# pyamg/pyamg

Measured on AMD Instinct MI355X. Metric: vcycle_iterations_per_sec, higher is better.
Workload: dtype f64; 1 GPU; 3D 7-pt Poisson 256^3 (16.7M dof) SA V-cycle, symmetric Gauss-Seidel, fp64; key=c3, n=16777216, nnz=117047296, levels=5, cycle=V(1,1), graph=True, parallelism=1 GPU, gs_order=fast, full=False

## Files before the change

### pyamg_amd/_build.py

```python
from __future__ import annotations

import os
import shutil
import subprocess
import sys
from concurrent.futures import ThreadPoolExecutor
from pathlib import Path

PKG = Path(__file__).resolve().parent
CSRC = PKG / "csrc"
LIB = PKG / "libpyamg_amd.so"
SOURCES = ["pamg_matrix.hip", "pamg_solver.hip", "pamg_capi.hip", "pamg_setup.hip", "pamg_schwarz.hip", "pamg_dist.hip", "pamg_aggregate.hip", "pamg_lane.hip", "pamg_line.hip", "pamg_kz.hip", "pamg_blane.hip", "pamg_block.hip", "pamg_renumber.hip", "pamg_krylov.hip", "pamg_schwarz_setup.hip", "pamg_classical.hip", "pamg_air.hip"]
HEADERS = ["pamg_common.h", "pamg_kernels.h", "pamg_tile_kernels.h", "pamg_tile_plan.h", "pamg_lane_plan.h", "pamg_lanem_plan.h", "pamg_schwarz_plan.h", "pamg_line_plan.h", "pamg_kz_plan.h", "pamg_blane_plan.h", "pamg_spg_plan.h", "pamg_stream_plan.h", "pamg_rowmask_map.h", "pamg_plan_vec.h", "pamg_host_threads.h", "pamg_dense_pinv.h", "pamg_classical.h", "pamg_air.h", "amg_core_bind.cpp", "../../include/pyamg_amd.h"]
FLAGS = ["--offload-arch=gfx950", "-O3", "-std=c++17", "-fPIC", "-ffp-contract=off",
         "-fno-fast-math", "-Wall", "-Wno-unused-function", "-Wno-unused-value", "-Wno-unused-result"]


def hipcc() -> str:
    for c in (os.environ.get("HIPCC"), shutil.which("hipcc"), "/opt/rocm/bin/hipcc"):
        if c and Path(c).exists():
            return c
    raise RuntimeError("hipcc not found (need ROCm's hipcc to build libpyamg_amd.so)")


def stale() -> bool:
    if not LIB.exists():
        return True
    try:
# ... 63 lines not shown
```

### pyamg_amd/csrc/pamg_common.h

```cpp
#pragma once
#include "pamg_host_threads.h"
#include <hip/hip_runtime.h>

#include <cstdint>
#include <cstdio>
#include <cstdlib>
#include <ctime>
#include <algorithm>
#include <atomic>
#include <cstring>
#include <thread>
#include <vector>

#include "../../include/pyamg_amd.h"

#define PAMG_STR2(x) #x
#define PAMG_STR(x) PAMG_STR2(x)
#define PAMG_HIP(expr)                                   \
    do {                                                 \
        hipError_t e__ = (expr);                         \
        if (e__ != hipSuccess) return (int)e__;          \
    } while (0)
#define PAMG_TRY(expr)                                   \
    do {                                                 \
// ... 200 lines not shown
    int sym_cap = 0;
    const void *sym_cap_kernel = nullptr;
    int zsym_cap = 0;
    const void *zsym_cap_kernel = nullptr;
    int csym_cap = 0;
    const void *csym_cap_kernel = nullptr;
    int sym_general_grid = 0;
    int sym_form = 0, sym_grid = 0;
    long long sym_launches = 0, sym_zero_launches = 0;
    int zero_plans = 0;
    int zero_merge = 0;
    struct pamg::LaneMSched *zplan[2] = {nullptr, nullptr};
    void *d_zw = nullptr;
    size_t zero_bytes = 0;
    long long zero_plan_launches = 0;
    int gs_correction = 0;
    long long correction_launches = 0;
    size_t bytes = 0;
};

struct pamg_schwarz_s;
struct pamg_solver_s;
struct pamg_csr_s;

namespace pamg {
int schwarz_sweep(pamg_schwarz_s *h, void *x, const void *b, int start, int stop, int step, hipStream_t s);
int schwarz_prepare(pamg_schwarz_s *h, int sweep);
int schwarz_error(pamg_schwarz_s *h, bool *error);
void schwarz_level_launches(pamg_schwarz_s *h);
int schwarz_blocks_device(int dtype, pamg_matrix_s *A, int nsub, const int *d_Sp, const int *d_Sj, int *d_Tp, void *d_Tx,
// ... 96 lines not shown
size_t lanem_part_bytes(const GsSchedule *g);
int lanem_info(const GsSchedule *g, int64_t *info, double *growth);
int lanem_levels(const GsSchedule *g, int64_t *out, int64_t cap, int64_t *n);
int lanem_sym_launch(pamg_matrix_s *A, GsSchedule *gf, GsSchedule *gb, void *x, const void *b, bool x_zero, hipStream_t s, bool acc = false);
int lanem_plan_info(const struct LaneMSched *t, int64_t *info, double *growth);
int build_zero_plan(pamg_matrix_s *A, int dir);
void free_zero_plans(pamg_matrix_s *A);
size_t zero_plan_bytes(const pamg_matrix_s *A);
bool zero_plans_ready(const pamg_matrix_s *A, const GsSchedule *gf, const GsSchedule *gb);
int lanem_zero_pair_launch(pamg_matrix_s *A, GsSchedule *gf, GsSchedule *gb, void *x, const void *b, bool acc, hipStream_t s);
int ensure_zero_parts(pamg_matrix_s *A, bool build);
void matrix_drop_zero_plans(pamg_matrix_s *A);
int gs_sweep_zero_pair(pamg_matrix_s *A, void *x, const void *b, hipStream_t s, bool *ran);
int gs_sweep_correction(pamg_matrix_s *A, void *x, const void *b, void *r, bool force, hipStream_t s, bool *ran);
constexpr int64_t GS_CORRECTION_MIN_ROWS = 16384;
int sym_fill_sentinels(void *p, int64_t n);
int sweep_error(pamg_matrix_s *A, bool *error);
inline size_t tsize(int dtype) { return dtype == PAMG_F64 ? 8 : 4; }

template <typename F>
inline void host_parallel(int64_t n, F fn, int64_t grain = 1 << 20)
{
    const unsigned hw = std::max(1u, std::min(32u, pamg::host_cpus()));
    const int nt = n < 2 * grain ? 1 : (int)std::min<int64_t>(hw, n / grain);
    if (nt <= 1) { fn((int64_t)0, n); return; }
    std::vector<std::thread> th;
    for (int t = 0; t < nt; ++t) {
        const int64_t lo = n * t / nt, hi = n * (t + 1) / nt;
        th.emplace_back([=] { fn(lo, hi); });
    }
// ... 19 lines not shown
```

### pyamg_amd/csrc/pamg_lane.hip

```cpp
#include "pamg_common.h"
#include "pamg_lane_plan.h"
#include "pamg_lanem_plan.h"
#include "pamg_tile_plan.h"

namespace pamg {

template <typename T> struct Sentinel;
template <> struct Sentinel<double> {
    using bits_t = unsigned long long;
    static constexpr bits_t value = 0x7FF8DEADBEEF5A5Aull;
    static __device__ __forceinline__ bits_t bits(double v) { return (bits_t)__double_as_longlong(v); }
};
template <> struct Sentinel<float> {
    using bits_t = unsigned int;
    static constexpr bits_t value = 0x7FC5BEEFu;
    static __device__ __forceinline__ bits_t bits(float v) { return __float_as_uint(v); }
};

template <typename T>
__global__ __launch_bounds__(BLK) void lane_fill_sentinel_kernel(T *xs, int64_t n)
{
    using B = typename Sentinel<T>::bits_t;
    B *p = reinterpret_cast<B *>(xs);
    for (int64_t i = (int64_t)blockIdx.x * BLK + threadIdx.x; i < n; i += (int64_t)gridDim.x * BLK) p[i] = Sentinel<T>::value;
// ... 301 lines not shown
    const void *cap_kernel = nullptr;
    size_t bytes = 0;
};

struct LaneMArgs {
    const int *cols;
    const double *vals;
    const LaneMRec *rec;
    const double *xold;
    double *y;
    double *xs;
    const double *b;
    unsigned *err;
    unsigned *ticket;
    int ngroups, nidle, use_gate;
    long long *prof;
    const unsigned short *sidx;
    const int *crid;
    const double *crd;
    int crows;
    double *w;
};

__global__ __launch_bounds__(BLK) void lanem_prepare_kernel(const double *__restrict__ x, double *__restrict__ xold, double *__restrict__ xs, int64_t n)
{
    unsigned long long *p = reinterpret_cast<unsigned long long *>(xs);
    for (int64_t i = (int64_t)blockIdx.x * BLK + threadIdx.x; i < n; i += (int64_t)gridDim.x * BLK) {
        xold[i] = x[i];
        p[i] = Sentinel<double>::value;
    }
// ... 272 lines not shown
    const T num = bv - s;
    T val = num * rd;
    if (!upd) val = xo;
    if (tail && rid >= 0) {
        __hip_atomic_store(a.xs + row, val, __ATOMIC_RELAXED, __HIP_MEMORY_SCOPE_AGENT);
        if constexpr (PH != 1) {
            if (upd) {
                if constexpr (ACC) a.y[row] = a.y[row] + val;
                else a.y[row] = val;
            }
        }
        if constexpr (WST) {
            if (upd) __hip_atomic_store(a.w + row, num, __ATOMIC_RELAXED, __HIP_MEMORY_SCOPE_AGENT);
        }
    }
}

template <int MODE, int RPW, int NREG, int Z = 0>
__global__ __launch_bounds__(BLK) void gs_lanem_kernel(const LaneMArgs a)
{
    const int lane = threadIdx.x & 63;
    const int wib = threadIdx.x >> 6;
    const int idle = (int)((((unsigned)blockIdx.x * LANE_WPB + (unsigned)wib) * 16u) % (unsigned)a.nidle);
    const int4 *rp = reinterpret_cast<const int4 *>(a.rec);
    const int gend = a.ngroups;
    __shared__ double c_lds[RPW == 0 ? LANE_WPB * LANEC_UMAX : 1];
    if constexpr (RPW == 0) {
        static_assert(RPW != 0 || MODE != 1, "the cluster layout has no ticket form");
        const int W = (int)gridDim.x * LANE_WPB;
        int g = __builtin_amdgcn_readfirstlane((int)blockIdx.x * LANE_WPB + wib);
// ... 28 lines not shown
                if (lane == 0) {
                    long long *o = a.prof + (size_t)g * 4;
                    o[0] = t0 | ((long long)(sp > 4095u ? 4095u : sp) << 52);
                    o[1] = t1; o[2] = t2; o[3] = wall_clock64();
                }
            } else {
                m_slots<RPW, NREG>(a, X, q0, q1, g, lane);
                m_gather<NREG>(a, X, idle);
                const double val = m_finish<RPW, NREG>(a, X, idle);
                m_publish<RPW, MODE, NREG, 0, Z == 1, Z == 2>(a, X, val);
            }
            q0 = n0; q1 = n1;
        }
    } else {
        __shared__ int sh_home;
        if (threadIdx.x == 0) {
            const unsigned me = (__builtin_amdgcn_s_getreg((3 << 11) | 20) & 0xF) + 1u;
            unsigned home = 0u;
            __hip_atomic_compare_exchange_strong(a.ticket + 1, &home, me, __ATOMIC_RELAXED, __ATOMIC_RELAXED, __HIP_MEMORY_SCOPE_AGENT);
            sh_home = (home == 0u || home == me) ? 1 : 0;
        }
        __syncthreads();
        if (!sh_home) return;
        unsigned tk = 0;
        if (lane == 0) tk = __hip_atomic_fetch_add(a.ticket, 1u, __ATOMIC_RELAXED, __HIP_MEMORY_SCOPE_AGENT);
        int g = (int)__builtin_amdgcn_readfirstlane(tk);
        if (g >= gend) return;
        if (lane == 0) tk = __hip_atomic_fetch_add(a.ticket, 1u, __ATOMIC_RELAXED, __HIP_MEMORY_SCOPE_AGENT);
        int g2 = (int)__builtin_amdgcn_readfirstlane(tk);
        int4 q0, q1;
        m_rec(rp, g, gend, q0, q1);
        while (true) {
            int4 n0, n1;
            m_rec(rp, g2, gend, n0, n1);
            unsigned tk3 = 0;
            if (g2 < gend && lane == 0) tk3 = __hip_atomic_fetch_add(a.ticket, 1u, __ATOMIC_RELAXED, __HIP_MEMORY_SCOPE_AGENT);
            m_slots<RPW, NREG>(a, X, q0, q1, g, lane);
            m_gather<NREG>(a, X, idle);
            const double val = m_finish<RPW, NREG>(a, X, idle);
            m_publish<RPW, MODE, NREG, 0, Z == 1, Z == 2>(a, X, val);
            if (g2 >= gend) break;
            g = g2; q0 = n0; q1 = n1;
            g2 = (int)__builtin_amdgcn_readfirstlane(tk3);
        }
    }
    }
}

struct LaneMSymArgs {
    LaneMArgs ph[2];
    double *hf[2];
    unsigned *sync;
    int wq[2], wr[2], wblk[2];
    int xzero;
};

template <int MODE>
__device__ __forceinline__ void m_wipe(double *w, int g, int G, int q, int r, int blk, int lane)
{
    if (g & (blk - 1)) return;
    const int g1 = g + blk < G ? g + blk : G;
    const int lo = g * q + (g < r ? g : r), hi = g1 * q + (g1 < r ? g1 : r);
    unsigned long long *p = reinterpret_cast<unsigned long long *>(w);
    for (int i = lo + lane; i < hi; i += 64) {
        if constexpr (MODE == 1) __hip_atomic_store(p + i, Sentinel<double>::value, __ATOMIC_RELAXED, __HIP_MEMORY_SCOPE_WORKGROUP);
        else __hip_atomic_store(p + i, Sentinel<double>::value, __ATOMIC_RELAXED, __HIP_MEMORY_SCOPE_AGENT);
    }
}

template <int MODE, int RPW, int NREG, int PH, int Z = 0>
__device__ __forceinline__ unsigned m_phase(const LaneMArgs &a, double *wipe, int wq, int wr, int wblk, unsigned *ticket, const bool xz, int lane, int wib, int idle, double *c_lds)
{
    const int4 *rp = reinterpret_cast<const int4 *>(a.rec);
    const int gend = a.ngroups;
    unsigned done = 0;
    if constexpr (RPW == 0) {
        static_assert(RPW != 0 || MODE != 1, "the cluster layout has no ticket form");
        const int W = (int)gridDim.x * LANE_WPB;
        int g = __builtin_amdgcn_readfirstlane((int)blockIdx.x * LANE_WPB + wib);
        if (g >= gend) return 0;
        int4 q = c_rec(rp, g, gend);
        for (; g < gend; g += W) {
            const int4 nq = c_rec(rp, g + W, gend);
            c_group<PH, Z && PH == 1, Z && PH == 2, Z == 2>(a, c_lds + wib * LANEC_UMAX, q, g, lane, idle, xz, PH == 2);
            m_wipe<MODE>(wipe, g, gend, wq, wr, wblk, lane);
            ++done;
// ... 7 lines not shown
        if (g >= gend) return 0;
        int4 q0, q1;
        m_rec(rp, g, gend, q0, q1);
        for (; g < gend; g += W) {
            int4 n0, n1;
            m_rec(rp, g + W, gend, n0, n1);
            m_slots<RPW, NREG>(a, X, q0, q1, g, lane);
            m_gather<NREG, Z && PH == 2, Z == 2 && PH == 1>(a, X, idle, xz, PH == 2);
            const double val = m_finish<RPW, NREG>(a, X, idle, nullptr, nullptr, xz);
            m_publish<RPW, MODE, NREG, PH, Z && PH == 1, Z == 2 && PH == 2>(a, X, val);
            m_wipe<MODE>(wipe, g, gend, wq, wr, wblk, lane);
            ++done;
            q0 = n0; q1 = n1;
        }
    } else {
        unsigned tk = 0;
        if (lane == 0) tk = __hip_atomic_fetch_add(ticket, 1u, __ATOMIC_RELAXED, __HIP_MEMORY_SCOPE_AGENT);
        int g = (int)__builtin_amdgcn_readfirstlane(tk);
        if (g >= gend) return 0;
        if (lane == 0) tk = __hip_atomic_fetch_add(ticket, 1u, __ATOMIC_RELAXED, __HIP_MEMORY_SCOPE_AGENT);
        int g2 = (int)__builtin_amdgcn_readfirstlane(tk);
        int4 q0, q1;
        m_rec(rp, g, gend, q0, q1);
        while (true) {
            int4 n0, n1;
            m_rec(rp, g2, gend, n0, n1);
            unsigned tk3 = 0;
            if (g2 < gend && lane == 0) tk3 = __hip_atomic_fetch_add(ticket, 1u, __ATOMIC_RELAXED, __HIP_MEMORY_SCOPE_AGENT);
            m_slots<RPW, NREG>(a, X, q0, q1, g, lane);
            m_gather<NREG, Z && PH == 2, Z == 2 && PH == 1>(a, X, idle, xz, PH == 2);
            const double val = m_finish<RPW, NREG>(a, X, idle, nullptr, nullptr, xz);
            m_publish<RPW, MODE, NREG, PH, Z && PH == 1, Z == 2 && PH == 2>(a, X, val);
            m_wipe<MODE>(wipe, g, gend, wq, wr, wblk, lane);
            ++done;
            if (g2 >= gend) break;
            g = g2; q0 = n0; q1 = n1;
            g2 = (int)__builtin_amdgcn_readfirstlane(tk3);
        }
    }
    }
    return done;
}

__device__ __forceinline__ void sym_phase_barrier(unsigned *counter, unsigned *err, unsigned *sh_done, unsigned done, unsigned total)
{
    asm volatile("s_waitcnt vmcnt(0)" ::: "memory");
    if ((threadIdx.x & 63) == 0 && done) atomicAdd(sh_done, done);
    __syncthreads();
    if (threadIdx.x == 0) {
        const unsigned mine = *sh_done;
        if (mine) __hip_atomic_fetch_add(counter, mine, __ATOMIC_RELAXED, __HIP_MEMORY_SCOPE_AGENT);
        unsigned spins = 0;
// ... 13 lines not shown
    __syncthreads();
    if (threadIdx.x == 0) {
        const unsigned left = __hip_atomic_fetch_add(sync + 1, 1u, __ATOMIC_RELAXED, __HIP_MEMORY_SCOPE_AGENT);
        if (left == gridDim.x - 1) {
            for (int k = 0; k < 5; ++k) __hip_atomic_store(sync + k, 0u, __ATOMIC_RELAXED, __HIP_MEMORY_SCOPE_AGENT);
            __hip_atomic_store(sync + 5, parity ^ 1u, __ATOMIC_RELAXED, __HIP_MEMORY_SCOPE_AGENT);
        }
    }
}

template <int MODE, int RPW, int NREG, int Z = 0>
__global__ __launch_bounds__(BLK) void gs_lanem_sym_kernel(const LaneMSymArgs a)
{
    __shared__ unsigned sh_done;
    __shared__ int sh_home;
    __shared__ double c_lds[RPW == 0 ? LANE_WPB * LANEC_UMAX : 1];
    const int lane = threadIdx.x & 63;
    const int wib = threadIdx.x >> 6;
    const int idle = (int)((((unsigned)blockIdx.x * LANE_WPB + (unsigned)wib) * 16u) % (unsigned)a.ph[0].nidle);
    const unsigned parity = __builtin_amdgcn_readfirstlane(__hip_atomic_load(a.sync + 5, __ATOMIC_RELAXED, __HIP_MEMORY_SCOPE_AGENT)) & 1u;
    if (threadIdx.x == 0) {
        sh_done = 0u;
        sh_home = 1;
        if constexpr (MODE == 1) {
            const unsigned me = (__builtin_amdgcn_s_getreg((3 << 11) | 20) & 0xF) + 1u;
            unsigned home = 0u;
            __hip_atomic_compare_exchange_strong(a.sync + 4, &home, me, __ATOMIC_RELAXED, __ATOMIC_RELAXED, __HIP_MEMORY_SCOPE_AGENT);
            sh_home = (home == 0u || home == me) ? 1 : 0;
        }
    }
    __syncthreads();
    if (sh_home) {
        double *hf = a.hf[parity], *hf_next = a.hf[parity ^ 1u];
        LaneMArgs p1 = a.ph[0], p2 = a.ph[1];
        p1.xs = hf; p1.y = nullptr;
        p2.xold = hf;
        const unsigned done = m_phase<MODE, RPW, NREG, 1, Z>(p1, p2.xs, a.wq[0], a.wr[0], a.wblk[0], a.sync + 2, a.xzero != 0, lane, wib, idle, c_lds);
        sym_phase_barrier(a.sync, p1.err, &sh_done, done, (unsigned)p1.ngroups);
        (void)m_phase<MODE, RPW, NREG, 2, Z>(p2, hf_next, a.wq[1], a.wr[1], a.wblk[1], a.sync + 3, false, lane, wib, idle, c_lds);
    }
    sym_leave(a.sync, parity);
}

namespace {

template <typename U>
int lane_upload(U **dst, const void *src, size_t bytes, size_t *total)
{
    *dst = nullptr;
    const size_t alloc = std::max<size_t>(bytes, 256) + 256;
    PAMG_HIP(hipMalloc((void **)dst, alloc));
    if (bytes && src) PAMG_HIP(hipMemcpy(*dst, src, bytes, hipMemcpyHostToDevice));
    if (total) *total += alloc;
    return PAMG_OK;
// ... 350 lines not shown
bool zero_plans_ready(const pamg_matrix_s *A, const GsSchedule *gf, const GsSchedule *gb)
{
    const LaneMSched *zf = A->zplan[0], *zb = A->zplan[1];
    if (A->zero_plans == 1 || !zf || !zb || !A->d_zw || !gf || !gb || !gf->lanem || !gb->lanem) return false;
    return zf->rpw == zb->rpw && zf->cluster == zb->cluster && zf->rpw == gf->lanem->rpw && zf->cluster == gf->lanem->cluster &&
           zb->rpw == gb->lanem->rpw && zb->cluster == gb->lanem->cluster && zf->ngroups >= 1 && zb->ngroups >= 1;
}

static void lanem_layout_args(const LaneMSched *t, LaneMArgs &a)
{
    a.cols = t->d_cols; a.vals = t->d_vals;
    a.rec = t->cluster ? reinterpret_cast<const LaneMRec *>(t->d_crec) : t->d_rec;
    a.sidx = t->d_sidx; a.crid = t->d_crid; a.crd = t->d_crd; a.crows = t->cluster;
}

static int lanem_launch_plan(pamg_matrix_s *A, GsSchedule *g, LaneMSched *t, void *x, const void *b, double *w, hipStream_t s, bool acc = false)
{
    if (!t || !g->d_xold) return PAMG_E_STATE;
    const int64_t n = A->nrows;
    LaneMArgs a;
    lanem_layout_args(t, a);
    a.use_gate = (A->lane_flags & 1) ? 1 : 0;
    a.xold = (const double *)g->d_xold; a.y = (double *)x; a.xs = (double *)g->d_xs; a.b = (const double *)b;
    a.w = w;
    a.err = g->d_sync + 1; a.ticket = g->d_sync + 20;
    a.ngroups = (int)t->ngroups;
    a.nidle = (int)std::max<int64_t>(1, std::min<int64_t>(n, 1 << 20));
    if (A->gs_prof && !t->d_prof && !t->cluster) {
        PAMG_HIP(hipMalloc((void **)&t->d_prof, (size_t)t->ngroups * 4 * sizeof(long long)));
        PAMG_HIP(hipMemset(t->d_prof, 0, (size_t)t->ngroups * 4 * sizeof(long long)));
    }
    a.prof = (A->gs_prof && !t->cluster) ? t->d_prof : nullptr;
    const int fgrid = (int)std::min<int64_t>(4096, (n + BLK - 1) / BLK);
    if (acc) hipLaunchKernelGGL((lane_fill_sentinel_kernel<double>), dim3(fgrid), dim3(BLK), 0, s, (double *)g->d_xs, n);
    else hipLaunchKernelGGL(lanem_prepare_kernel, dim3(fgrid), dim3(BLK), 0, s, (const double *)x, (double *)g->d_xold, (double *)g->d_xs, n);
    PAMG_HIP(hipGetLastError());
    const bool xcd = !t->cluster && (A->gran_xcd == 1 || (A->gran_xcd == 0 && lane_one_xcd(A, g) && A->nrows <= 8192));
    static const int nreg_env = [] { const char *e = getenv("PAMG_LANEM_NREG"); return e ? atoi(e) : 0; }();
    const bool all_regs = t->rpw == 1 && (nreg_env ? nreg_env == 8 : A->nrows <= 131072);
    const void *k = t->cluster  ? (const void *)gs_lanem_kernel<0, 0, 8>
                  : t->rpw == 2 ? (xcd ? (const void *)gs_lanem_kernel<1, 2, 4> : (const void *)gs_lanem_kernel<0, 2, 4>)
                  : all_regs    ? (xcd ? (const void *)gs_lanem_kernel<1, 1, 8> : (const void *)gs_lanem_kernel<0, 1, 8>)
                                : (xcd ? (const void *)gs_lanem_kernel<1, 1, 2> : (const void *)gs_lanem_kernel<0, 1, 2>);
    if (w)
        k = t->cluster  ? (const void *)gs_lanem_kernel<0, 0, 8, 1>
          : t->rpw == 2 ? (xcd ? (const void *)gs_lanem_kernel<1, 2, 4, 1> : (const void *)gs_lanem_kernel<0, 2, 4, 1>)
          : all_regs    ? (xcd ? (const void *)gs_lanem_kernel<1, 1, 8, 1> : (const void *)gs_lanem_kernel<0, 1, 8, 1>)
                        : (xcd ? (const void *)gs_lanem_kernel<1, 1, 2, 1> : (const void *)gs_lanem_kernel<0, 1, 2, 1>);
    if (acc)
        k = t->cluster  ? (const void *)gs_lanem_kernel<0, 0, 8, 2>
          : t->rpw == 2 ? (xcd ? (const void *)gs_lanem_kernel<1, 2, 4, 2> : (const void *)gs_lanem_kernel<0, 2, 4, 2>)
          : all_regs    ? (xcd ? (const void *)gs_lanem_kernel<1, 1, 8, 2> : (const void *)gs_lanem_kernel<0, 1, 8, 2>)
// ... 51 lines not shown
    hipLaunchKernelGGL((lane_fill_sentinel_kernel<double>), dim3(fgrid), dim3(BLK), 0, 0, (double *)p, n);
    PAMG_HIP(hipGetLastError());
    PAMG_HIP(hipDeviceSynchronize());
    return PAMG_OK;
}

int lanem_sym_launch(pamg_matrix_s *A, GsSchedule *gf, GsSchedule *gb, void *x, const void *b, bool x_zero, hipStream_t s, bool acc)
{
    LaneMSched *tf = gf->lanem, *tb = gb->lanem;
    if (!tf || !tb || !A->d_sym_hf[0] || !A->d_sym_hf[1] || !A->d_sym_hb || !A->d_sym_sync) return PAMG_E_STATE;
    if (acc && !zero_plans_ready(A, gf, gb)) return PAMG_E_UNSUPPORTED;
    if (acc) x_zero = true;
    const bool zero = x_zero && zero_plans_ready(A, gf, gb);
    if (zero) { tf = A->zplan[0]; tb = A->zplan[1]; }
    const int64_t n = A->nrows;
    auto one_xcd = [&](const GsSchedule *g) { return !g->lanem->cluster && (A->gran_xcd == 1 || (A->gran_xcd == 0 && lane_one_xcd(A, g) && A->nrows <= 8192)); };
    const bool xcd = one_xcd(gf);
    if (xcd != one_xcd(gb) || tf->rpw != tb->rpw || tf->cluster != tb->cluster || tf->ngroups < 1 || tb->ngroups < 1) return PAMG_E_UNSUPPORTED;
    LaneMSymArgs a;
    LaneMSched *ts2[2] = {tf, tb};
    for (int p = 0; p < 2; ++p) {
        LaneMSched *t = ts2[p];
        LaneMArgs &q = a.ph[p];
        lanem_layout_args(t, q);
        q.use_gate = (A->lane_flags & 1) ? 1 : 0;
        q.b = (const double *)b;
        q.w = nullptr;
        q.err = gf->d_sync + 1; q.ticket = nullptr;
        q.ngroups = (int)t->ngroups;
        q.nidle = (int)std::max<int64_t>(1, std::min<int64_t>(n, 1 << 20));
        q.prof = nullptr;
        a.wq[p] = (int)(n / t->ngroups); a.wr[p] = (int)(n % t->ngroups);
        a.wblk[p] = 1;
        while ((int64_t)a.wblk[p] * n < 64 * t->ngroups && a.wblk[p] < (1 << 20)) a.wblk[p] *= 2;
    }
    a.ph[0].xold = (const double *)x; a.ph[0].y = nullptr;     a.ph[0].xs = nullptr;
    a.ph[1].xold = nullptr;           a.ph[1].y = (double *)x; a.ph[1].xs = (double *)A->d_sym_hb;
    if (zero) { a.ph[0].w = (double *)A->d_zw; a.ph[1].b = (const double *)A->d_zw; }
    a.hf[0] = (double *)A->d_sym_hf[0]; a.hf[1] = (double *)A->d_sym_hf[1];
    a.sync = A->d_sym_sync;
    a.xzero = x_zero ? 1 : 0;
    static const int nreg_env = [] { const char *e = getenv("PAMG_LANEM_NREG"); return e ? atoi(e) : 0; }();
    const bool all_regs = tf->rpw == 1 && (nreg_env ? nreg_env == 8 : A->nrows <= 131072);
    const void *k = tf->cluster  ? (const void *)gs_lanem_sym_kernel<0, 0, 8>
// ... 174 lines not shown
```

### pyamg_amd/csrc/pamg_matrix.hip

```cpp
#include "pamg_host_threads.h"
#include <algorithm>
#include <atomic>
#include <mutex>
#include <climits>
#include <new>
#include <thread>

#include "pamg_kernels.h"
#include "pamg_tile_kernels.h"
#include "pamg_tile_plan.h"
#include "pamg_stream_plan.h"

using namespace pamg;

namespace {

constexpr int PAD = 8;

std::mutex g_sched_mu;

template <typename U>
int upload(U **dptr, const U *h, size_t n, size_t *bytes)
{
    const size_t sz = (n + PAD) * sizeof(U);
// ... 1061 lines not shown
    int r0, r1, rs;
    if (A->gs_order != 1 || A->gs_mode != 0 || A->R != A->C || A->point_twin_unfit || !point_twin_bounds(A, g, r0, r1, rs)) return PAMG_OK;
    static std::mutex twin_mu;
    {
        std::lock_guard<std::mutex> lk(twin_mu);
        if (A->point_twin_unfit) return PAMG_OK;
        if (!A->point_twin) {
            PhaseTimer pt_("point twin of a block operator", A->nnz);
            std::vector<unsigned char> hAx((size_t)A->nnz * tsize(A->dtype));
            if (A->nnz) PAMG_HIP(hipMemcpy(hAx.data(), A->d_Ax, hAx.size(), hipMemcpyDeviceToHost));
            pamg_matrix_s *T = nullptr;
            const int st = pamg_matrix_create(&T, A->dtype, PAMG_CSR, (int)A->nrows, (int)A->ncols, 1, 1, A->h_Ap.data(), A->h_Aj.data(), hAx.data());
            if (st != PAMG_OK) { A->point_twin_unfit = true; return st == PAMG_E_UNSUPPORTED || st == PAMG_E_ARG ? PAMG_OK : st; }
            T->gs_order = 1;
            T->lane_L = A->lane_L; T->lane_G = A->lane_G; T->lane_flags = A->lane_flags; T->lane_merge = A->lane_merge; T->line_scan = A->line_scan;
            T->lane_wide = A->lane_wide; T->lanem_rpw = A->lanem_rpw; T->lanem_cluster = A->lanem_cluster; T->lanem_ahead10 = A->lanem_ahead10; T->gran_xcd = A->gran_xcd;
            A->point_twin = T;
            { std::lock_guard<std::mutex> lk2(g_sched_mu); A->bytes += T->bytes; A->point_twin_bytes = T->bytes; }
        }
    }
    GsSchedule *tg = nullptr;
    PAMG_TRY(get_schedule(A->point_twin, r0, r1, rs, &tg));
    PAMG_TRY(ensure_parts(A->point_twin, tg, false));
    if (!tg->lane && !tg->lanem && !tg->line) {
        std::lock_guard<std::mutex> lk(twin_mu);
        A->point_twin_unfit = true;
    }
    return PAMG_OK;
}

int ensure_parts(pamg_matrix_s *A, GsSchedule *g, bool block_gs)
// ... 876 lines not shown
        case 18: if (value < 0 || value > 1) return PAMG_E_ARG; A->tile_part = value; break;
        case 19: A->use_idx16 = value != 0; return PAMG_OK;
        case 20: if (value != 0 && (value < 64 || value > 2048)) return PAMG_E_ARG; A->gs_cap = value & ~3; break;
        case 24: if (value < 0 || value > 1) return PAMG_E_ARG; A->gs_order = value; return PAMG_OK;
        case 25: if (value != 0 && value != 4 && value != 8 && value != 16 && value != 32 && value != 64) return PAMG_E_ARG; A->lane_L = value; break;
        case 26: if (value < 0) return PAMG_E_ARG; A->lane_G = value; matrix_drop_point_twin(A); return PAMG_OK;
        case 27: if (value < 0 || value > 1) return PAMG_E_ARG; A->lane_wide = value; matrix_drop_point_twin(A); return PAMG_OK;
        case 33: if (value < 0 || value > 8) return PAMG_E_ARG; A->lane_merge = value; break;
        case 35: if (value < 0 || value > 2) return PAMG_E_ARG; A->lanem_rpw = value; break;
        case 38: if (value != 0 && value != 1 && value != 4 && value != 8) return PAMG_E_ARG; A->lanem_cluster = value; break;
        case 36: if (value < 0 || value > 98304) return PAMG_E_ARG; A->lds_pad = value & ~15; return PAMG_OK;
        case 34: if (value < 1 || value > 400) return PAMG_E_ARG; A->lanem_ahead10 = value; matrix_drop_point_twin(A); return PAMG_OK;
        case 37: if (value < 0 || value > 1) return PAMG_E_ARG; A->sym_fused = value; return PAMG_OK;
        case 39: if (value < 0 || value > 2) return PAMG_E_ARG; A->zero_plans = value; if (value == 1) matrix_drop_zero_plans(A); return PAMG_OK;
        case 40: if (value != 0 && (value < 2 || value > 16)) return PAMG_E_ARG; A->zero_merge = value; matrix_drop_zero_plans(A); return PAMG_OK;
        case 41: if (value < 0 || value > 2) return PAMG_E_ARG; A->gs_correction = value; return PAMG_OK;
        case 30:
            if (value < 0 || value > 2) return PAMG_E_ARG;
            A->line_scan = value;
            matrix_drop_point_twin(A);
            for (int k = 0; k < 4; ++k) if (A->gs[k]) A->gs[k]->line_unfit = false;
            return PAMG_OK;
        case 31: if (value != 2 && value != 4 && value != 8) return PAMG_E_ARG; A->rowmask_kz = value; return PAMG_OK;
        case 32: if (value < 0 || value > 7) return PAMG_E_ARG; A->rowmask_flags = value; return PAMG_OK;
        case 28: if (value < 0 || value > 15 || (value & 6)) return PAMG_E_ARG; A->lane_flags = value; matrix_drop_point_twin(A); return PAMG_OK;
        default: return PAMG_E_ARG;
    }
    if (key == 25 || key == 33 || key == 35 || key == 38) {
        matrix_drop_point_twin(A);
        matrix_drop_zero_plans(A);
// ... 353 lines not shown
```

### pyamg_amd/multilevel.py

```python
from __future__ import annotations

import ctypes as C
from typing import List, Optional

import numpy as np

from . import _capi as capi
from .hierarchy import HierarchySpec, SmootherSpec, SparseOp, extract

__all__ = ["DeviceMatrix", "DeviceMultilevelSolver"]


class DeviceMatrix:

    def __init__(self, op: SparseOp):
        lib = capi.lib()
        self.op = op
        self.dtype = np.dtype(op.dtype)
        R, Cc = op.blocksize
        h = C.c_void_p()
        capi.check(lib.pamg_matrix_create(
            C.byref(h), capi.dtype_code(op.dtype), capi.BSR if op.fmt == "bsr" else capi.CSR,
            op.shape[0] // R, op.shape[1] // Cc, R, Cc,
            capi.ptr(op.indptr), capi.ptr(op.indices), capi.ptr(op.data)), "pamg_matrix_create")
# ... 115 lines not shown
        a = (C.c_int64 * 8)()
        capi.check(capi.lib().pamg_matrix_kz_info(self.handle, which, a), "pamg_matrix_kz_info")
        return dict(zip(("lanes_per_line", "slots_per_lane", "groups", "dependency_levels", "widest_level_groups", "launch_grid", "bytes"), list(a)[:7]))

    def lane_profile(self, which=0):
        n = C.c_int64(0)
        lib = capi.lib()
        capi.check(lib.pamg_matrix_lane_profile(self.handle, which, None, 0, C.byref(n)), "pamg_matrix_lane_profile")
        out = np.zeros((n.value, 4), dtype=np.int64)
        if n.value:
            capi.check(lib.pamg_matrix_lane_profile(self.handle, which, C.c_void_p(out.ctypes.data), n.value, C.byref(n)), "pamg_matrix_lane_profile")
        return out

    def tune(self, lds_entries=None, nnz_per_lane=None, max_rows=None, flow_cap=None, gs_mode=None, gran_cap=None, gran_xcd=None, stream_flags=None, gs_prof=None,
             tile_G=None, tile_W=None, tile_cap=None, tile_default=None, tile_D=None, tile_Q=None, tile_part=None, idx16=None, gs_cap=None, val8=None, rowgather=None, rowpat=None,
             gs_order=None, lane_L=None, lane_G=None, lane_wide=None, lane_flags=None, line_scan=None, rowmask_kz=None, rowmask_flags=None, lane_merge=None, lanem_ahead=None, lanem_rpw=None, lds_pad=None, sym_fused=None, lanem_cluster=None, zero_plans=None, zero_merge=None, gs_correction=None):
        lib = capi.lib()
        for key, v in ((0, lds_entries), (1, nnz_per_lane), (2, max_rows), (3, flow_cap), (5, gs_mode), (6, gran_cap), (7, gran_xcd), (8, stream_flags), (11, gs_prof),
                       (12, tile_G), (13, tile_W), (14, tile_cap), (15, tile_default), (16, tile_D), (17, tile_Q), (18, tile_part), (19, idx16), (20, gs_cap), (21, val8), (22, rowgather), (23, rowpat),
                       (24, gs_order), (25, lane_L), (26, lane_G), (27, lane_wide), (28, lane_flags), (30, line_scan), (31, rowmask_kz), (32, rowmask_flags), (33, lane_merge), (34, lanem_ahead), (35, lanem_rpw), (36, lds_pad), (37, sym_fused), (38, lanem_cluster), (39, zero_plans), (40, zero_merge), (41, gs_correction)):
            if v is not None:
                capi.check(lib.pamg_matrix_tune(self.handle, key, int(v)), "pamg_matrix_tune")

    def spmv(self, mode, x, y, b=None, c=0.0, stream=None, part=None):
        if part is not None:
            capi.check(capi.lib().pamg_matrix_spmv_part(self.handle, int(part), mode, x.ptr, b.ptr if b is not None else None,
                                                        float(c), y.ptr, stream), "pamg_matrix_spmv_part")
            return
        capi.check(capi.lib().pamg_matrix_spmv(self.handle, mode, x.ptr, b.ptr if b is not None else None,
                                               float(c), y.ptr, stream), "pamg_matrix_spmv")

    def split_ranges(self, n_owned_cols: int):
        capi.check(capi.lib().pamg_matrix_split_ranges(self.handle, int(n_owned_cols)), "pamg_matrix_split_ranges")

    def resid_sumsq(self, x, b, out, stream=None):
# ... 570 lines not shown
```

Before: 95.99 cycles/s.

## Batch group tickets per workgroup in single-XCD lane-merge GS kernels

Replaces the per-wave global atomic ticket claim in the single-XCD lanem Gauss-Seidel path with a workgroup-level scheme. One lane draws a global ticket covering a batch of WPB*m groups, shares it through an LDS ring, and waves walk strided groups within the batch. The aim is fewer agent-scope atomics on the ticket counter, at the cost of LDS spin-waiting and intra-workgroup coupling. With the default auto batch m=1, each ticket covers 4 groups (one per wave). The path only applies to small matrices (coarse levels, or when gran_xcd is forced).

```diff
diff --git a/pyamg_amd/_build.py b/pyamg_amd/_build.py
--- a/pyamg_amd/_build.py
+++ b/pyamg_amd/_build.py
@@ -11,7 +11,7 @@
 CSRC = PKG / "csrc"
 LIB = PKG / "libpyamg_amd.so"
 SOURCES = ["pamg_matrix.hip", "pamg_solver.hip", "pamg_capi.hip", "pamg_setup.hip", "pamg_schwarz.hip", "pamg_dist.hip", "pamg_aggregate.hip", "pamg_lane.hip", "pamg_line.hip", "pamg_kz.hip", "pamg_blane.hip", "pamg_block.hip", "pamg_renumber.hip", "pamg_krylov.hip", "pamg_schwarz_setup.hip", "pamg_classical.hip", "pamg_air.hip"]
-HEADERS = ["pamg_common.h", "pamg_kernels.h", "pamg_tile_kernels.h", "pamg_tile_plan.h", "pamg_lane_plan.h", "pamg_lanem_plan.h", "pamg_schwarz_plan.h", "pamg_line_plan.h", "pamg_kz_plan.h", "pamg_blane_plan.h", "pamg_spg_plan.h", "pamg_stream_plan.h", "pamg_rowmask_map.h", "pamg_plan_vec.h", "pamg_host_threads.h", "pamg_dense_pinv.h", "pamg_classical.h", "pamg_air.h", "amg_core_bind.cpp", "../../include/pyamg_amd.h"]
+HEADERS = ["pamg_common.h", "pamg_kernels.h", "pamg_tile_kernels.h", "pamg_tile_plan.h", "pamg_lane_plan.h", "pamg_lanem_plan.h", "pamg_schwarz_plan.h", "pamg_line_plan.h", "pamg_kz_plan.h", "pamg_blane_plan.h", "pamg_spg_plan.h", "pamg_stream_plan.h", "pamg_rowmask_map.h", "pamg_plan_vec.h", "pamg_host_threads.h", "pamg_dense_pinv.h", "pamg_classical.h", "pamg_air.h", "pamg_xcd_batch.h", "amg_core_bind.cpp", "../../include/pyamg_amd.h"]
 FLAGS = ["--offload-arch=gfx950", "-O3", "-std=c++17", "-fPIC", "-ffp-contract=off",
          "-fno-fast-math", "-Wall", "-Wno-unused-function", "-Wno-unused-value", "-Wno-unused-result"]
 
diff --git a/pyamg_amd/csrc/pamg_common.h b/pyamg_amd/csrc/pamg_common.h
--- a/pyamg_amd/csrc/pamg_common.h
+++ b/pyamg_amd/csrc/pamg_common.h
@@ -238,6 +238,7 @@
     void *d_zw = nullptr;
     size_t zero_bytes = 0;
     long long zero_plan_launches = 0;
+    int xcd_batch = 0;
     int gs_correction = 0;
     long long correction_launches = 0;
     size_t bytes = 0;
@@ -364,6 +365,7 @@
 int gs_sweep_zero_pair(pamg_matrix_s *A, void *x, const void *b, hipStream_t s, bool *ran);
 int gs_sweep_correction(pamg_matrix_s *A, void *x, const void *b, void *r, bool force, hipStream_t s, bool *ran);
 constexpr int64_t GS_CORRECTION_MIN_ROWS = 16384;
+constexpr int XCD_BATCH_AUTO = 1;
 int sym_fill_sentinels(void *p, int64_t n);
 int sweep_error(pamg_matrix_s *A, bool *error);
 inline size_t tsize(int dtype) { return dtype == PAMG_F64 ? 8 : 4; }
diff --git a/pyamg_amd/csrc/pamg_lane.hip b/pyamg_amd/csrc/pamg_lane.hip
--- a/pyamg_amd/csrc/pamg_lane.hip
+++ b/pyamg_amd/csrc/pamg_lane.hip
@@ -2,6 +2,7 @@
 #include "pamg_lane_plan.h"
 #include "pamg_lanem_plan.h"
 #include "pamg_tile_plan.h"
+#include "pamg_xcd_batch.h"
 
 namespace pamg {
 
@@ -339,6 +340,7 @@
     unsigned *err;
     unsigned *ticket;
     int ngroups, nidle, use_gate;
+    int batch;
     long long *prof;
     const unsigned short *sidx;
     const int *crid;
@@ -641,6 +643,113 @@
             if (upd) __hip_atomic_store(a.w + row, num, __ATOMIC_RELAXED, __HIP_MEMORY_SCOPE_AGENT);
         }
     }
+}
+
+static_assert(XB_WPB == LANE_WPB, "pamg_xcd_batch.h walks a workgroup of LANE_WPB waves");
+struct XbShared {
+    unsigned long long slot[XB_RING];
+    unsigned claim;
+    unsigned have[XB_WPB];
+};
+struct XbWalk {
+    long long base;
+    unsigned j;
+    int m;
+    unsigned dj, dtk;
+    bool drew;
+};
+
+__device__ __forceinline__ void xb_init(XbShared &S)
+{
+    for (int k = 0; k < XB_RING; ++k) S.slot[k] = 0ull;
+    S.claim = 0u;
+    for (int w = 0; w < XB_WPB; ++w) S.have[w] = 0u;
+}
+
+__device__ __forceinline__ bool xb_spin_out(unsigned &spins, unsigned *err)
+{
+    __builtin_amdgcn_s_sleep(1);
+    if ((++spins & 1023u) == 0 && (spins > (1u << 21) || __hip_atomic_load(err, __ATOMIC_RELAXED, __HIP_MEMORY_SCOPE_AGENT))) {
+        __hip_atomic_store(err, 1u, __ATOMIC_RELAXED, __HIP_MEMORY_SCOPE_AGENT);
+        return true;
+    }
+    return false;
+}
+
+__device__ __forceinline__ void xb_flush(XbShared &S, XbWalk &W)
+{
+    if (W.drew) {
+        __hip_atomic_store(&S.slot[xb_slot(W.dj)], xb_pack(W.dj, W.dtk), __ATOMIC_RELAXED, __HIP_MEMORY_SCOPE_WORKGROUP);
+        W.drew = false;
+    }
+}
+
+__device__ __forceinline__ void xb_try_draw(XbShared &S, XbWalk &W, unsigned *ticket, unsigned *err, unsigned J)
+{
+    unsigned seen = J;
+    if (!__hip_atomic_compare_exchange_strong(&S.claim, &seen, J + 1u, __ATOMIC_RELAXED, __ATOMIC_RELAXED, __HIP_MEMORY_SCOPE_WORKGROUP)) return;
+    unsigned spins = 0;
+    while (J > 0u && !xb_holds(__hip_atomic_load(&S.slot[xb_slot(J - 1u)], __ATOMIC_RELAXED, __HIP_MEMORY_SCOPE_WORKGROUP), J - 1u))
+        if (xb_spin_out(spins, err)) break;
+    const unsigned need = xb_reads_needed(J);
+    for (int w = 0; w < XB_WPB; ++w)
+        while (__hip_atomic_load(&S.have[w], __ATOMIC_RELAXED, __HIP_MEMORY_SCOPE_WORKGROUP) < need)
+            if (xb_spin_out(spins, err)) break;
+    W.dtk = __hip_atomic_fetch_add(ticket, 1u, __ATOMIC_RELAXED, __HIP_MEMORY_SCOPE_AGENT);
+    W.dj = J;
+    W.drew = true;
+}
+
+__device__ __forceinline__ unsigned xb_read(XbShared &S, unsigned *err, unsigned J, int wib)
+{
+    unsigned spins = 0;
+    unsigned long long v;
+    while (!xb_holds(v = __hip_atomic_load(&S.slot[xb_slot(J)], __ATOMIC_RELAXED, __HIP_MEMORY_SCOPE_WORKGROUP), J))
+        if (xb_spin_out(spins, err)) return 0xFFFFFFFFu;
+    __hip_atomic_store(&S.have[wib], J + 1u, __ATOMIC_RELAXED, __HIP_MEMORY_SCOPE_WORKGROUP);
+    return xb_ticket(v);
+}
+
+__device__ __forceinline__ int xb_cross(XbShared &S, XbWalk &W, unsigned *ticket, unsigned *err, int gend, int lane, int wib)
+{
+    int n = gend;
+    unsigned j = W.j;
+    int blo = 0;
+    if (lane == 0) {
+        while (true) {
+            xb_flush(S, W);
+            const unsigned t = xb_read(S, err, j + 1u, wib);
+            ++j;
+            const long long base = xb_batch_base(t, W.m);
+            if (base >= (long long)gend) break;
+            blo = (int)base;
+            xb_try_draw(S, W, ticket, err, j + (unsigned)XB_AHEAD);
+            const long long g = xb_group(base, wib, 0);
+            if (g < (long long)gend) { n = (int)g; break; }
+        }
+    }
+    W.j = __builtin_amdgcn_readfirstlane(j);
+    W.base = (long long)__builtin_amdgcn_readfirstlane(blo);
+    return __builtin_amdgcn_readfirstlane(n);
+}
+
+__device__ __forceinline__ int xb_start(XbShared &S, XbWalk &W, unsigned *ticket, unsigned *err, int m, int gend, int lane, int wib)
+{
+    W.m = m < 1 ? 1 : m; W.drew = false; W.dj = 0u; W.dtk = 0u; W.base = 0; W.j = 0xFFFFFFFFu;
+    if (lane == 0) {
+        for (unsigned J = 0; J < (unsigned)XB_AHEAD; ++J) {
+            xb_try_draw(S, W, ticket, err, J);
+            xb_flush(S, W);
+        }
+    }
+    return xb_cross(S, W, ticket, err, gend, lane, wib);
+}
+
+__device__ __forceinline__ int xb_next(XbShared &S, XbWalk &W, unsigned *ticket, unsigned *err, int g, int gend, int lane, int wib)
+{
+    const long long n = xb_next_in_batch((long long)g, W.base, W.m, (long long)gend);
+    if (n >= 0) return (int)n;
+    return xb_cross(S, W, ticket, err, gend, lane, wib);
 }
 
 template <int MODE, int RPW, int NREG, int Z = 0>
@@ -699,7 +808,9 @@
         }
     } else {
         __shared__ int sh_home;
+        __shared__ XbShared sh_xb;
         if (threadIdx.x == 0) {
+            xb_init(sh_xb);
             const unsigned me = (__builtin_amdgcn_s_getreg((3 << 11) | 20) & 0xF) + 1u;
             unsigned home = 0u;
             __hip_atomic_compare_exchange_strong(a.ticket + 1, &home, me, __ATOMIC_RELAXED, __ATOMIC_RELAXED, __HIP_MEMORY_SCOPE_AGENT);
@@ -707,26 +818,22 @@
         }
         __syncthreads();
         if (!sh_home) return;
-        unsigned tk = 0;
-        if (lane == 0) tk = __hip_atomic_fetch_add(a.ticket, 1u, __ATOMIC_RELAXED, __HIP_MEMORY_SCOPE_AGENT);
-        int g = (int)__builtin_amdgcn_readfirstlane(tk);
+        XbWalk wk;
+        int g = xb_start(sh_xb, wk, a.ticket, a.err, a.batch, gend, lane, wib);
         if (g >= gend) return;
-        if (lane == 0) tk = __hip_atomic_fetch_add(a.ticket, 1u, __ATOMIC_RELAXED, __HIP_MEMORY_SCOPE_AGENT);
-        int g2 = (int)__builtin_amdgcn_readfirstlane(tk);
         int4 q0, q1;
         m_rec(rp, g, gend, q0, q1);
         while (true) {
+            const int g2 = xb_next(sh_xb, wk, a.ticket, a.err, g, gend, lane, wib);
             int4 n0, n1;
             m_rec(rp, g2, gend, n0, n1);
-            unsigned tk3 = 0;
-            if (g2 < gend && lane == 0) tk3 = __hip_atomic_fetch_add(a.ticket, 1u, __ATOMIC_RELAXED, __HIP_MEMORY_SCOPE_AGENT);
             m_slots<RPW, NREG>(a, X, q0, q1, g, lane);
             m_gather<NREG>(a, X, idle);
+            if (lane == 0) xb_flush(sh_xb, wk);
             const double val = m_finish<RPW, NREG>(a, X, idle);
             m_publish<RPW, MODE, NREG, 0, Z == 1, Z == 2>(a, X, val);
             if (g2 >= gend) break;
             g = g2; q0 = n0; q1 = n1;
-            g2 = (int)__builtin_amdgcn_readfirstlane(tk3);
         }
     }
     }
@@ -743,9 +850,9 @@
 template <int MODE>
 __device__ __forceinline__ void m_wipe(double *w, int g, int G, int q, int r, int blk, int lane)
 {
-    if (g & (blk - 1)) return;
-    const int g1 = g + blk < G ? g + blk : G;
-    const int lo = g * q + (g < r ? g : r), hi = g1 * q + (g1 < r ? g1 : r);
+    int lo, hi;
+    xb_wipe_range(g, G, q, r, blk, lo, hi);
+    if (lo >= hi) return;
     unsigned long long *p = reinterpret_cast<unsigned long long *>(w);
     for (int i = lo + lane; i < hi; i += 64) {
         if constexpr (MODE == 1) __hip_atomic_store(p + i, Sentinel<double>::value, __ATOMIC_RELAXED, __HIP_MEMORY_SCOPE_WORKGROUP);
@@ -754,7 +861,7 @@
 }
 
 template <int MODE, int RPW, int NREG, int PH, int Z = 0>
-__device__ __forceinline__ unsigned m_phase(const LaneMArgs &a, double *wipe, int wq, int wr, int wblk, unsigned *ticket, const bool xz, int lane, int wib, int idle, double *c_lds)
+__device__ __forceinline__ unsigned m_phase(const LaneMArgs &a, double *wipe, int wq, int wr, int wblk, unsigned *ticket, XbShared *xb, const bool xz, int lane, int wib, int idle, double *c_lds)
 {
     const int4 *rp = reinterpret_cast<const int4 *>(a.rec);
     const int gend = a.ngroups;
@@ -792,28 +899,24 @@
             q0 = n0; q1 = n1;
         }
     } else {
-        unsigned tk = 0;
-        if (lane == 0) tk = __hip_atomic_fetch_add(ticket, 1u, __ATOMIC_RELAXED, __HIP_MEMORY_SCOPE_AGENT);
-        int g = (int)__builtin_amdgcn_readfirstlane(tk);
+        XbWalk wk;
+        int g = xb_start(*xb, wk, ticket, a.err, a.batch, gend, lane, wib);
         if (g >= gend) return 0;
-        if (lane == 0) tk = __hip_atomic_fetch_add(ticket, 1u, __ATOMIC_RELAXED, __HIP_MEMORY_SCOPE_AGENT);
-        int g2 = (int)__builtin_amdgcn_readfirstlane(tk);
         int4 q0, q1;
         m_rec(rp, g, gend, q0, q1);
         while (true) {
+            const int g2 = xb_next(*xb, wk, ticket, a.err, g, gend, lane, wib);
             int4 n0, n1;
             m_rec(rp, g2, gend, n0, n1);
-            unsigned tk3 = 0;
-            if (g2 < gend && lane == 0) tk3 = __hip_atomic_fetch_add(ticket, 1u, __ATOMIC_RELAXED, __HIP_MEMORY_SCOPE_AGENT);
             m_slots<RPW, NREG>(a, X, q0, q1, g, lane);
             m_gather<NREG, Z && PH == 2, Z == 2 && PH == 1>(a, X, idle, xz, PH == 2);
+            if (lane == 0) xb_flush(*xb, wk);
             const double val = m_finish<RPW, NREG>(a, X, idle, nullptr, nullptr, xz);
             m_publish<RPW, MODE, NREG, PH, Z && PH == 1, Z == 2 && PH == 2>(a, X, val);
             m_wipe<MODE>(wipe, g, gend, wq, wr, wblk, lane);
             ++done;
             if (g2 >= gend) break;
             g = g2; q0 = n0; q1 = n1;
-            g2 = (int)__builtin_amdgcn_readfirstlane(tk3);
         }
     }
     }
@@ -857,6 +960,7 @@
 {
     __shared__ unsigned sh_done;
     __shared__ int sh_home;
+    __shared__ XbShared sh_xb[MODE == 1 ? 2 : 1];
     __shared__ double c_lds[RPW == 0 ? LANE_WPB * LANEC_UMAX : 1];
     const int lane = threadIdx.x & 63;
     const int wib = threadIdx.x >> 6;
@@ -865,6 +969,7 @@
     if (threadIdx.x == 0) {
         sh_done = 0u;
         sh_home = 1;
+        if constexpr (MODE == 1) { xb_init(sh_xb[0]); xb_init(sh_xb[1]); }
         if constexpr (MODE == 1) {
             const unsigned me = (__builtin_amdgcn_s_getreg((3 << 11) | 20) & 0xF) + 1u;
             unsigned home = 0u;
@@ -878,9 +983,9 @@
         LaneMArgs p1 = a.ph[0], p2 = a.ph[1];
         p1.xs = hf; p1.y = nullptr;
         p2.xold = hf;
-        const unsigned done = m_phase<MODE, RPW, NREG, 1, Z>(p1, p2.xs, a.wq[0], a.wr[0], a.wblk[0], a.sync + 2, a.xzero != 0, lane, wib, idle, c_lds);
+        const unsigned done = m_phase<MODE, RPW, NREG, 1, Z>(p1, p2.xs, a.wq[0], a.wr[0], a.wblk[0], a.sync + 2, &sh_xb[0], a.xzero != 0, lane, wib, idle, c_lds);
         sym_phase_barrier(a.sync, p1.err, &sh_done, done, (unsigned)p1.ngroups);
-        (void)m_phase<MODE, RPW, NREG, 2, Z>(p2, hf_next, a.wq[1], a.wr[1], a.wblk[1], a.sync + 3, false, lane, wib, idle, c_lds);
+        (void)m_phase<MODE, RPW, NREG, 2, Z>(p2, hf_next, a.wq[1], a.wr[1], a.wblk[1], a.sync + 3, &sh_xb[1], false, lane, wib, idle, c_lds);
     }
     sym_leave(a.sync, parity);
 }
@@ -1261,6 +1366,17 @@
     a.sidx = t->d_sidx; a.crid = t->d_crid; a.crd = t->d_crd; a.crows = t->cluster;
 }
 
+static bool lanem_one_xcd(const pamg_matrix_s *A, const GsSchedule *g)
+{
+    const LaneMSched *t = g->lanem;
+    if (!t || t->cluster) return false;
+    if (A->gran_xcd == 1) return true;
+    if (A->gran_xcd != 0 || !lane_one_xcd(A, g)) return false;
+    return A->nrows <= 8192;
+}
+
+static int lanem_xcd_batch(const pamg_matrix_s *A) { return A->xcd_batch > 0 ? std::min(A->xcd_batch, XB_MAX_M) : XCD_BATCH_AUTO; }
+
 static int lanem_launch_plan(pamg_matrix_s *A, GsSchedule *g, LaneMSched *t, void *x, const void *b, double *w, hipStream_t s, bool acc = false)
 {
     if (!t || !g->d_xold) return PAMG_E_STATE;
@@ -1282,7 +1398,8 @@
     if (acc) hipLaunchKernelGGL((lane_fill_sentinel_kernel<double>), dim3(fgrid), dim3(BLK), 0, s, (double *)g->d_xs, n);
     else hipLaunchKernelGGL(lanem_prepare_kernel, dim3(fgrid), dim3(BLK), 0, s, (const double *)x, (double *)g->d_xold, (double *)g->d_xs, n);
     PAMG_HIP(hipGetLastError());
-    const bool xcd = !t->cluster && (A->gran_xcd == 1 || (A->gran_xcd == 0 && lane_one_xcd(A, g) && A->nrows <= 8192));
+    const bool xcd = lanem_one_xcd(A, g);
+    a.batch = lanem_xcd_batch(A);
     static const int nreg_env = [] { const char *e = getenv("PAMG_LANEM_NREG"); return e ? atoi(e) : 0; }();
     const bool all_regs = t->rpw == 1 && (nreg_env ? nreg_env == 8 : A->nrows <= 131072);
     const void *k = t->cluster  ? (const void *)gs_lanem_kernel<0, 0, 8>
@@ -1364,7 +1481,7 @@
     const bool zero = x_zero && zero_plans_ready(A, gf, gb);
     if (zero) { tf = A->zplan[0]; tb = A->zplan[1]; }
     const int64_t n = A->nrows;
-    auto one_xcd = [&](const GsSchedule *g) { return !g->lanem->cluster && (A->gran_xcd == 1 || (A->gran_xcd == 0 && lane_one_xcd(A, g) && A->nrows <= 8192)); };
+    auto one_xcd = [&](const GsSchedule *g) { return lanem_one_xcd(A, g); };
     const bool xcd = one_xcd(gf);
     if (xcd != one_xcd(gb) || tf->rpw != tb->rpw || tf->cluster != tb->cluster || tf->ngroups < 1 || tb->ngroups < 1) return PAMG_E_UNSUPPORTED;
     LaneMSymArgs a;
@@ -1378,6 +1495,7 @@
         q.w = nullptr;
         q.err = gf->d_sync + 1; q.ticket = nullptr;
         q.ngroups = (int)t->ngroups;
+        q.batch = lanem_xcd_batch(A);
         q.nidle = (int)std::max<int64_t>(1, std::min<int64_t>(n, 1 << 20));
         q.prof = nullptr;
         a.wq[p] = (int)(n / t->ngroups); a.wr[p] = (int)(n % t->ngroups);
diff --git a/pyamg_amd/csrc/pamg_matrix.hip b/pyamg_amd/csrc/pamg_matrix.hip
--- a/pyamg_amd/csrc/pamg_matrix.hip
+++ b/pyamg_amd/csrc/pamg_matrix.hip
@@ -1099,7 +1099,7 @@
             if (st != PAMG_OK) { A->point_twin_unfit = true; return st == PAMG_E_UNSUPPORTED || st == PAMG_E_ARG ? PAMG_OK : st; }
             T->gs_order = 1;
             T->lane_L = A->lane_L; T->lane_G = A->lane_G; T->lane_flags = A->lane_flags; T->lane_merge = A->lane_merge; T->line_scan = A->line_scan;
-            T->lane_wide = A->lane_wide; T->lanem_rpw = A->lanem_rpw; T->lanem_cluster = A->lanem_cluster; T->lanem_ahead10 = A->lanem_ahead10; T->gran_xcd = A->gran_xcd;
+            T->lane_wide = A->lane_wide; T->lanem_rpw = A->lanem_rpw; T->lanem_cluster = A->lanem_cluster; T->lanem_ahead10 = A->lanem_ahead10; T->gran_xcd = A->gran_xcd; T->xcd_batch = A->xcd_batch;
             A->point_twin = T;
             { std::lock_guard<std::mutex> lk2(g_sched_mu); A->bytes += T->bytes; A->point_twin_bytes = T->bytes; }
         }
@@ -2006,6 +2006,7 @@
         case 37: if (value < 0 || value > 1) return PAMG_E_ARG; A->sym_fused = value; return PAMG_OK;
         case 39: if (value < 0 || value > 2) return PAMG_E_ARG; A->zero_plans = value; if (value == 1) matrix_drop_zero_plans(A); return PAMG_OK;
         case 40: if (value != 0 && (value < 2 || value > 16)) return PAMG_E_ARG; A->zero_merge = value; matrix_drop_zero_plans(A); return PAMG_OK;
+        case 42: if (value < 0 || value > 16) return PAMG_E_ARG; A->xcd_batch = value; matrix_drop_point_twin(A); return PAMG_OK;
         case 41: if (value < 0 || value > 2) return PAMG_E_ARG; A->gs_correction = value; return PAMG_OK;
         case 30:
             if (value < 0 || value > 2) return PAMG_E_ARG;
diff --git a/pyamg_amd/csrc/pamg_xcd_batch.h b/pyamg_amd/csrc/pamg_xcd_batch.h
--- /dev/null
+++ b/pyamg_amd/csrc/pamg_xcd_batch.h
@@ -0,0 +1,45 @@
+#pragma once
+
+#if defined(__HIPCC__)
+#define PAMG_XB_HD __host__ __device__ __forceinline__
+#else
+#define PAMG_XB_HD inline
+#endif
+
+namespace pamg {
+
+constexpr int XB_WPB = 4;
+constexpr int XB_RING = 8;
+constexpr int XB_AHEAD = 2;
+constexpr int XB_MAX_M = 16;
+
+PAMG_XB_HD int xb_batch_groups(int m) { return XB_WPB * m; }
+
+PAMG_XB_HD long long xb_num_batches(long long ngroups, int m) { return (ngroups + xb_batch_groups(m) - 1) / xb_batch_groups(m); }
+
+PAMG_XB_HD long long xb_batch_base(unsigned ticket, int m) { return (long long)ticket * (long long)xb_batch_groups(m); }
+
+PAMG_XB_HD long long xb_group(long long base, int w, int k) { return base + (long long)w + (long long)k * XB_WPB; }
+
+PAMG_XB_HD long long xb_next_in_batch(long long g, long long base, int m, long long ngroups)
+{
+    const long long n = g + XB_WPB;
+    return (n < base + xb_batch_groups(m) && n < ngroups) ? n : -1;
+}
+
+PAMG_XB_HD int xb_slot(unsigned j) { return (int)(j % (unsigned)XB_RING); }
+PAMG_XB_HD unsigned long long xb_pack(unsigned j, unsigned ticket) { return ((unsigned long long)(j + 1u) << 32) | (unsigned long long)ticket; }
+PAMG_XB_HD bool xb_holds(unsigned long long v, unsigned j) { return (unsigned)(v >> 32) == j + 1u; }
+PAMG_XB_HD unsigned xb_ticket(unsigned long long v) { return (unsigned)(v & 0xFFFFFFFFull); }
+PAMG_XB_HD unsigned xb_reads_needed(unsigned j) { return j >= (unsigned)XB_RING ? j - (unsigned)XB_RING + 1u : 0u; }
+
+PAMG_XB_HD void xb_wipe_range(int g, int G, int q, int r, int blk, int &lo, int &hi)
+{
+    lo = hi = 0;
+    if (g & (blk - 1)) return;
+    const int g1 = g + blk < G ? g + blk : G;
+    lo = g * q + (g < r ? g : r);
+    hi = g1 * q + (g1 < r ? g1 : r);
+}
+
+}
diff --git a/pyamg_amd/multilevel.py b/pyamg_amd/multilevel.py
--- a/pyamg_amd/multilevel.py
+++ b/pyamg_amd/multilevel.py
@@ -153,11 +153,11 @@
 
     def tune(self, lds_entries=None, nnz_per_lane=None, max_rows=None, flow_cap=None, gs_mode=None, gran_cap=None, gran_xcd=None, stream_flags=None, gs_prof=None,
              tile_G=None, tile_W=None, tile_cap=None, tile_default=None, tile_D=None, tile_Q=None, tile_part=None, idx16=None, gs_cap=None, val8=None, rowgather=None, rowpat=None,
-             gs_order=None, lane_L=None, lane_G=None, lane_wide=None, lane_flags=None, line_scan=None, rowmask_kz=None, rowmask_flags=None, lane_merge=None, lanem_ahead=None, lanem_rpw=None, lds_pad=None, sym_fused=None, lanem_cluster=None, zero_plans=None, zero_merge=None, gs_correction=None):
+             gs_order=None, lane_L=None, lane_G=None, lane_wide=None, lane_flags=None, line_scan=None, rowmask_kz=None, rowmask_flags=None, lane_merge=None, lanem_ahead=None, lanem_rpw=None, lds_pad=None, sym_fused=None, lanem_cluster=None, zero_plans=None, zero_merge=None, gs_correction=None, xcd_batch=None):
         lib = capi.lib()
         for key, v in ((0, lds_entries), (1, nnz_per_lane), (2, max_rows), (3, flow_cap), (5, gs_mode), (6, gran_cap), (7, gran_xcd), (8, stream_flags), (11, gs_prof),
                        (12, tile_G), (13, tile_W), (14, tile_cap), (15, tile_default), (16, tile_D), (17, tile_Q), (18, tile_part), (19, idx16), (20, gs_cap), (21, val8), (22, rowgather), (23, rowpat),
-                       (24, gs_order), (25, lane_L), (26, lane_G), (27, lane_wide), (28, lane_flags), (30, line_scan), (31, rowmask_kz), (32, rowmask_flags), (33, lane_merge), (34, lanem_ahead), (35, lanem_rpw), (36, lds_pad), (37, sym_fused), (38, lanem_cluster), (39, zero_plans), (40, zero_merge), (41, gs_correction)):
+                       (24, gs_order), (25, lane_L), (26, lane_G), (27, lane_wide), (28, lane_flags), (30, line_scan), (31, rowmask_kz), (32, rowmask_flags), (33, lane_merge), (34, lanem_ahead), (35, lanem_rpw), (36, lds_pad), (37, sym_fused), (38, lanem_cluster), (39, zero_plans), (40, zero_merge), (41, gs_correction), (42, xcd_batch)):
             if v is not None:
                 capi.check(lib.pamg_matrix_tune(self.handle, key, int(v)), "pamg_matrix_tune")
 
```

After: 96.11 cycles/s, median of 6. About the same (+0.1%).
